# kirilllzaitsev/vision_mtl

Hardware: AMD Instinct MI355X
Metric: images/sec fwd+bwd, basic model 128x256 (higher is better)
Workload: dtype f32

## Files before the change

### include/vmtl.h

```cpp
#ifndef VMTL_H
#define VMTL_H

#ifdef __cplusplus
extern "C" {
#endif

#define VMTL_ACT_NONE 0
#define VMTL_ACT_RELU 1
#define VMTL_ACT_HSWISH 2
#define VMTL_ACT_HSIGMOID 3
#define VMTL_ACT_SIGMOID 4

#define VMTL_PREC_FP32 0
#define VMTL_PREC_BF16 1

const char* vmtl_version(void);
const char* vmtl_last_error_string(void);
int vmtl_reload_env(void);
int vmtl_timestamp(long long* out, void* stream);


int vmtl_conv2d_fwd(const float* x, const float* wp, const float* bias, float* y, float* stats,
                    int B, int H, int W, int Cs, int Ho, int Wo, int ldy, int Nw, int Cout,
                    int KH, int KW, int stride, int pad, int act, int shuffle, void* stream);
// ... 63 lines not shown
int vmtl_unpack_up2(const float* slabs, float* grad, int Cout, int Cos, int C0, int Cin, int nslabs, void* stream);

int vmtl_conv2d_wgrad_splits(int M, int Nw, int Ktot);
int vmtl_conv2d_wgrad(const float* x, const float* dy, float* slabs, int splits, int B, int H, int W, int Cs,
                      int Ho, int Wo, int ldy, int Nw, int KH, int KW, int stride, int pad, void* stream);
int vmtl_conv2d_wgrad_p(const float* x, const float* dy, float* slabs, int splits, int B, int H, int W, int Cs,
                        int Ho, int Wo, int ldy, int Nw, int KH, int KW, int stride, int pad, int precision,
                        void* stream);

int vmtl_conv3x3_wgrad_small_supported(int Cs, int ldy, int W);
int vmtl_conv3x3_wgrad_small_slabs(int B, int H, int W);
int vmtl_conv3x3_wgrad_small(const float* x, const float* dy, float* slabs, int nslabs, int B, int H, int W, int Cs,
                             int ldy, int Nw, void* stream);


int vmtl_conv3x3_small_supported(int Cs, int Nw);
int vmtl_conv3x3_small_tiles(int B, int H, int W);
int vmtl_conv3x3_small_stat_rows(int B, int H, int W);
int vmtl_conv3x3_small_stat_block(int B, int H, int W);
int vmtl_conv3x3_small(const float* x, const float* x2, const float* pa, const float* pb, const float* pc,
                       int act_in, float* a_out, const float* wp, const float* bias, float* y, float* yb, int Ca,
                       float* stats, int ep_mode, const float* ez_x, const float* ez_mean, const float* ez_invstd,
                       const float* ez_gamma, const float* ez_beta, int ez_act, int B, int H, int W, int Cs, int ldy,
                       int Nw, int Cout, void* stream);

int vmtl_conv3x3_halo_supported(int B, int H, int W, int Cs, int ldy, int Nw);
int vmtl_conv3x3_halo_stat_rows(int B, int H, int W);
int vmtl_conv3x3_halo_stat_block(int B, int H, int W);
int vmtl_conv3x3_halo(const float* x, const float* pa, const float* pc, int act_in, float* a_out, const float* wp,
                      const float* bias, float* y, float* stats, int ep_mode, const float* ez_x, const float* ez_mean,
                      const float* ez_invstd, const float* ez_gamma, const float* ez_beta, int ez_act, int B, int H,
                      int W, int Cs, int ldy, int Nw, int Cout, void* stream);

int vmtl_dwconv_fwd(const float* x, const float* wp, float* y, int B, int H, int W, int Cs, int Ho, int Wo,
                    int K, int stride, int pad, void* stream);
int vmtl_dwconv_bn_stats_rows(int M, int Cs);
int vmtl_dwconv_bn_stats_block(int M, int Cs);
int vmtl_dwconv_bn_fwd(const float* x, const float* coef_a, const float* coef_c, int act, const float* wp, float* y,
                       float* a_out, float* partial, int B, int H, int W, int Cs, int Ho, int Wo, int K, int stride,
                       int pad, void* stream);
int vmtl_dwconv_bwd_data(const float* dy, const float* wp, float* dx, int B, int H, int W, int Cs, int Ho,
                         int Wo, int K, int stride, int pad, void* stream);
int vmtl_dwconv_bwd_data_add(const float* dy, const float* wp, const float* addend, float* dx, int B, int H, int W,
                             int Cs, int Ho, int Wo, int K, int stride, int pad, void* stream);
int vmtl_dwconv_bwd_weight_rows(int M, int Cs);
int vmtl_dwconv_bwd_weight(const float* x, const float* dy, float* partial, float* dw, int B, int H, int W,
                           int C, int Cs, int Ho, int Wo, int K, int stride, int pad, void* stream);

int vmtl_pack_weights(const float* src, float* dst, int R1, int R0, int T, int C, int Cs, long long sr1,
                      long long sr0, long long st, long long sc, int flip, void* stream);
int vmtl_pack_weights_scaled(const float* src, float* dst, int R1, int R0, int T, int C, int Cs, long long sr1,
                             long long sr0, long long st, long long sc, int flip, const float* scale, int sstride,
                             int smode, void* stream);
int vmtl_unpack_weights_stitch(const float* packed, float* grad, const float* w, const float* scale, int sstride,
                               float* ds, float* work, int R0, int T, int C, int Cs, int nslabs, long long slab_stride,
                               int reduce_all, void* stream);
int vmtl_pack_desc_bytes(void);
int vmtl_pack_weights_batch(const void* descs, int n, long long total, void* stream);
int vmtl_pack_weights_slice(const float* src, float* dst, int R0, int T, int C, int group, long long sr0,
                            long long st, long long sc, int flip, void* stream);
int vmtl_unpack_weights(const float* packed, float* grad, int R1, int R0, int T, int C, int Cs,
                        long long sr1, long long sr0, long long st, long long sc, int flip, int nslabs,
                        long long slab_stride, void* stream);

int vmtl_reduce_rows(int M);
int vmtl_bn_stats(const float* x, int M, int C, int Cs, float* partial, int nblk_from_conv,
                  int rows_per_blk_from_conv, float eps, float momentum, float* running_mean, float* running_var, long long* num_batches_tracked,
                  float* save_mean, float* save_invstd, void* stream);
int vmtl_bn_eval_stats(const float* running_mean, const float* running_var, int C, int Cs, float eps,
                       float* save_mean, float* save_invstd, void* stream);
int vmtl_bn_stats_coef(const float* x, int M, int C, int Cs, float* partial, int nblk_from_conv,
                       int rows_per_blk_from_conv, float eps, float momentum, float* running_mean, float* running_var,
                       long long* num_batches_tracked, float* save_mean, float* save_invstd, const float* gamma,
                       const float* beta, float* coef_a, float* coef_c, void* stream);
int vmtl_bn_eval_stats_coef(const float* running_mean, const float* running_var, int C, int Cs, float eps,
                            float* save_mean, float* save_invstd, const float* gamma, const float* beta,
                            float* coef_a, float* coef_c, void* stream);
int vmtl_bn_eval_desc_bytes(void);
int vmtl_bn_eval_stats_batch(const void* descs, int n, int max_cs, void* stream);
int vmtl_bn_apply(const float* x, const float* mean, const float* invstd, const float* gamma,
                  const float* beta, const float* mul, const float* res, float* y, long long M, int C,
                  int Cs, int act, void* stream);
int vmtl_bn_fuse_max_rows(void);
int vmtl_bn_apply_fused(const float* x, const float* partial, int nblk, int rows_per_blk, float eps, float momentum,
                        float* running_mean, float* running_var, long long* num_batches_tracked, float* save_mean,
                        float* save_invstd, const float* gamma, const float* beta, const float* mul, const float* res,
                        float* y, long long M, int C, int Cs, int act, void* stream);
int vmtl_bn_bwd(const float* x, const float* dy, const float* mean, const float* invstd, const float* gamma,
                const float* beta, const float* mul, float* dmul, float* partial, float* sum_dz,
                float* sum_dzx, float* dx, int M, int C, int Cs, int act, int training, void* stream);
int vmtl_bn_bwd_finalize(const float* partial, int nblk, int M, int C, int Cs, float* sum_dz, float* sum_dzx,
                         const float* mean, const float* invstd, const float* gamma, int training, float* coef_a,
                         float* coef_b, float* coef_c, void* stream);
int vmtl_bn_bwd_apply(const float* x, const float* dz, const float* mean, const float* invstd, const float* gamma,
                      const float* sum_dz, const float* sum_dzx, float* dx, int M, int C, int Cs, int training,
                      void* stream);

int vmtl_bn_act_pool2_fwd(const float* x, const float* mean, const float* invstd, const float* gamma,
                          const float* beta, float* y, int B, int H, int W, int C, int Cs, int act, void* stream);
int vmtl_bn_act_pool2_bwd(const float* x, const float* dyp, const float* mean, const float* invstd,
                          const float* gamma, const float* beta, float* partial, float* sum_dz, float* sum_dzx,
                          float* dx, int B, int H, int W, int C, int Cs, int act, int training, void* stream);

int vmtl_conv2d_dgrad_s2_supported(int K, int pad);
long long vmtl_conv2d_dgrad_s2_ws(int B, int H, int W, int Cs, int Ho, int Wo, int ldy, int K, int pad);
long long vmtl_pack_dgrad_s2_size(int Cin, int ldy, int K, int pad);
int vmtl_pack_dgrad_s2(const float* w, float* dst, int Cout, int Cin, int ldy, int K, int pad, void* stream);
int vmtl_conv2d_dgrad_s2(const float* dy, const float* wp, float* dx, float* ws, int B, int H, int W, int Cs, int Ho,
                         int Wo, int ldy, int Cin, int K, int pad, void* stream);
int vmtl_conv2d_dgrad_s2_p(const float* dy, const float* wp, float* dx, float* ws, int B, int H, int W, int Cs, int Ho,
                           int Wo, int ldy, int Cin, int K, int pad, int precision, void* stream);
int vmtl_bn_act_pool3s2_fwd(const float* x, const float* mean, const float* invstd, const float* gamma,
                            const float* beta, float* a_out, float* y, unsigned char* idx, int B, int H, int W, int C,
                            int Cs, int act, void* stream);
int vmtl_bn_act_pool3s2_bwd(const float* x, const float* dskip, const float* dyp, const unsigned char* idx,
                            const float* mean, const float* invstd, const float* gamma, const float* beta, float* dz,
                            float* partial, float* sum_dz, float* sum_dzx, float* dx, int B, int H, int W, int C, int Cs,
                            int act, int training, void* stream);
int vmtl_bn_add_act_fwd(const float* z, const float* mean_a, const float* invstd_a, const float* gamma_a,
                        const float* beta_a, const float* res, const float* zd, const float* mean_b, const float* invstd_b,
                        const float* gamma_b, const float* beta_b, float* y, int M, int C, int Cs, int act, void* stream);
int vmtl_bn_add_act_bwd(const float* z, const float* mean_a, const float* invstd_a, const float* gamma_a,
                        const float* beta_a, const float* res, const float* zd, const float* mean_b, const float* invstd_b,
                        const float* gamma_b, const float* beta_b, const float* dy, float* g, float* partial,
                        float* sum_dz_a, float* sum_dzx_a, float* sum_dz_b, float* sum_dzx_b, float* dz, float* dzd, int M,
                        int C, int Cs, int act, int training, void* stream);

int vmtl_colsum(const float* a, const float* b, int M, int C, int Cs, int mode, int reduce_all,
                float* partial, float* out, void* stream);

int vmtl_concat2(const float* a, int Ha, int Wa, int Ca, int Csa, int upa, int oha, int owa,
                 const float* b, int Hb, int Wb, int Cb, int Csb, int upb, int ohb, int owb, float* y,
                 int B, int H, int W, int Cd, void* stream);
int vmtl_concat2_bwd(const float* dy, float* dx, int B, int H, int W, int Cd, int c_off, int Hs, int Ws,
                     int C, int Cs, int up, int oh, int ow, void* stream);
int vmtl_maxpool2_fwd(const float* x, float* y, int B, int H, int W, int Cs, void* stream);
int vmtl_maxpool2_bwd(const float* x, const float* dy, float* dx, int B, int H, int W, int Cs, void* stream);
int vmtl_bilinear_up2_fwd(const float* x, float* y, int B, int H, int W, int Cs, void* stream);
int vmtl_bilinear_up2_bwd(const float* dy, float* dx, int B, int H, int W, int Cs, void* stream);
int vmtl_spatial_mean(const float* x, float* y, int B, int HW, int Cs, void* stream);
int vmtl_channel_bcast(const float* x, const float* s, float* y, int B, int HW, int Cs, int mode, void* stream);
int vmtl_channel_scale_bwd_s(const float* x, const float* dy, float* ds, int B, int HW, int Cs, void* stream);
int vmtl_fc_max_rows(void);
int vmtl_fc_fwd(const float* a, int a_parts, long long a_part_stride, float a_scale, const float* a_z, int a_act,
                float* a_out, const float* w, const float* bias, float* z, float* y, int M, int K, int N, int lda,
                int ldw, int ldy, int act, void* stream);
int vmtl_fc_wgrad(const float* x, int x_parts, long long x_part_stride, float x_scale, const float* dyo, int dy_parts,
                  long long dy_part_stride, const float* zo, float* dw, float* db, int M, int K, int N, int lda, int ldn,
                  int act, void* stream);
int vmtl_hw_reduce_parts(int B, int HW, int Cs);
int vmtl_hw_reduce(const float* x, const float* y, float* part, int B, int HW, int Cs, void* stream);
int vmtl_channel_scale_add(const float* x, const float* s, const float* t, float t_scale, float* y, int B, int HW,
                           int Cs, void* stream);
int vmtl_stitch(const float* x, const float* w, float* y, long long M, int C, int Cs, int wstride, void* stream);
int vmtl_stitch_bwd(const float* x, const float* dy, const float* w, float* dx, float* partial, float* dw, int M,
                    int C, int Cs, int wstride, int reduce_all, void* stream);
int vmtl_eltwise(const float* a, const float* b, float* y, int mode, long long total, void* stream);
int vmtl_add_n(const float* a, const float* b, const float* c, const float* d, float* y, long long total, void* stream);
int vmtl_axpby(const float* a, const float* b, float* y, float wa, float wb, long long total, void* stream);
int vmtl_fill_zero(float* p, long long n, void* stream);
int vmtl_argmax_channels(const float* z, long long* out, int B, int HW, int C, long long sb, long long sc,
                         long long sp, void* stream);
int vmtl_nchw_to_nhwc(const float* x, float* y, int B, int C, int HW, int Cs, int Cw, void* stream);
int vmtl_nhwc_to_nchw(const float* x, float* y, int B, int C, int HW, int Cs, void* stream);
int vmtl_hwc_to_nhwc_pad(const float* x, float* y, long long P, int C, int Cs, float scale, void* stream);
#define VMTL_DEPTH_U16 0
#define VMTL_DEPTH_I32 1
int vmtl_nyuv2_resize_parts(int B, int Hi, int Wi, int Ho, int Wo, int depth_dtype);
int vmtl_nyuv2_resize(const void* img, const void* mask, const void* depth, int depth_dtype, float* img_out,
                      long long* mask_out, float* depth_out, float* part, int B, int Hi, int Wi, int Ho, int Wo,
                      float max_depth, void* stream);

long long vmtl_ce_workspace_bytes(long long P);
int vmtl_ce_fwd(const float* logits, const long long* target, float* loss, void* workspace, int B, int HW,
                int C, long long sb, long long sc, long long sp, void* stream);
int vmtl_ce_fwd_argmax(const float* logits, const long long* target, float* loss, void* workspace,
                       long long* argmax, int B, int HW, int C, long long sb, long long sc, long long sp,
                       void* stream);
int vmtl_ce_bwd(const float* logits, const long long* target, const float* grad_out, float* dlogits, int B,
                int HW, int C, long long sb, long long sc, long long sp, void* stream);
int vmtl_ce_bwd_strided(const float* logits, const long long* target, const float* grad_out, float* dlogits, int B,
                        int HW, int C, long long sb, long long sc, long long sp, long long dsb, long long dsc,
                        long long dsp, void* stream);
long long vmtl_silog_workspace_bytes(long long P);
int vmtl_silog_fwd(const float* pred, const float* target, float min_depth, float* loss, float* stats,
                   void* workspace, long long P, void* stream);
int vmtl_silog_bwd(const float* pred, const float* target, const float* stats, const float* grad_out,
                   float min_depth, float* dpred, long long P, void* stream);
int vmtl_l1_fwd(const float* pred, const float* target, float* loss, void* workspace, long long P, void* stream);
int vmtl_l1_bwd(const float* pred, const float* target, const float* grad_out, float* dpred, long long P,
                void* stream);

int vmtl_confusion_matrix(const long long* pred, const long long* target, int* cm, long long P, int C,
                          void* stream);
int vmtl_segm_metrics(const int* cm, int C, float beta, float* out, void* stream);

int vmtl_adam_step(float* p, const float* g, float* m, float* v, const float* step_ptr, float lr, float b1,
                   float b2, float eps, float weight_decay, float grad_scale, long long n, void* stream);

#ifdef __cplusplus
}
#endif
#endif
```

### vision_mtl_amd/csrc/fc.hip

```cpp
#include "common.h"

struct FcP {
  const float* a;
  const float* a_z;
  const float* w;
  const float* bias;
  float* a_out;
  float* z;
  float* y;
  long long a_part_stride;
  float a_scale;
  int a_parts, a_act;
  int M, K, N, lda, ldw, ldy, act;
};

#define FC_WAVES 8
#define FC_UNROLL 4

template <int MT>
__global__ __launch_bounds__(FC_WAVES * 64) void fc_kernel(FcP p) {
  __shared__ f32x4 red[FC_WAVES][MT][64];
  const int tid = threadIdx.x, lane = tid & 63, wv = tid >> 6;
  const int l15 = lane & 15, lq = lane >> 4;
  const int n0 = blockIdx.x * 16;
  const int n = n0 + l15;
  f32x4 acc[MT];
#pragma unroll
  for (int t = 0; t < MT; ++t) acc[t] = (f32x4){0.f, 0.f, 0.f, 0.f};
  const int nchunks = (p.K + 15) >> 4;
  const bool wvec = (p.ldw & 3) == 0;
  for (int c0 = wv; c0 < nchunks; c0 += FC_WAVES * FC_UNROLL) {
    f32x4 fb[FC_UNROLL], fa[FC_UNROLL][MT];
#pragma unroll
    for (int u = 0; u < FC_UNROLL; ++u) {
      const int c = c0 + u * FC_WAVES;
      const int k4 = c * 16 + lq * 4;
      fb[u] = (f32x4){0.f, 0.f, 0.f, 0.f};
      if (c < nchunks && n < p.N && k4 < p.K) {
        const float* wp = p.w + (size_t)n * p.ldw + k4;
        if (wvec && k4 + 3 < p.K) {
          fb[u] = *reinterpret_cast<const f32x4*>(wp);
        } else {
#pragma unroll
          for (int e = 0; e < 4; ++e)
            if (k4 + e < p.K) fb[u][e] = wp[e];
        }
      }
#pragma unroll
      for (int t = 0; t < MT; ++t) {
        const int m = t * 16 + l15;
        f32x4 v = {0.f, 0.f, 0.f, 0.f};
        if (c < nchunks && m < p.M && k4 < p.lda) {
          const float* ap = p.a + (size_t)m * p.lda + k4;
          v = *reinterpret_cast<const f32x4*>(ap);
          for (int s = 1; s < p.a_parts; ++s) v += *reinterpret_cast<const f32x4*>(ap + s * p.a_part_stride);
          v *= p.a_scale;
          if (p.a_out != nullptr && (c % (int)gridDim.x) == (int)blockIdx.x)
            *reinterpret_cast<f32x4*>(p.a_out + (size_t)m * p.lda + k4) = v;
          if (p.a_z != nullptr) {
            const f32x4 zv = *reinterpret_cast<const f32x4*>(p.a_z + (size_t)m * p.lda + k4);
#pragma unroll
            for (int e = 0; e < 4; ++e) v[e] *= act_grad(zv[e], p.a_act);
          }
        }
        fa[u][t] = v;
      }
    }
#pragma unroll
    for (int u = 0; u < FC_UNROLL; ++u)
#pragma unroll
      for (int t = 0; t < MT; ++t)
#pragma unroll
        for (int e = 0; e < 4; ++e)
          acc[t] = __builtin_amdgcn_mfma_f32_16x16x4f32(fa[u][t][e], fb[u][e], acc[t], 0, 0, 0);
  }
#pragma unroll
  for (int t = 0; t < MT; ++t) red[wv][t][lane] = acc[t];
  __syncthreads();
  if (tid >= 512) return;
  const int ln = tid & 63, rg = (tid >> 6) & 3, rt = tid >> 8;
  const int col = ln & 15, row = 4 * (ln >> 4) + rg;
  const int nn = n0 + col;
  if (nn >= p.ldy) return;
  const float bv = (p.bias != nullptr && nn < p.N) ? p.bias[nn] : 0.f;
  for (int t = rt; t < MT; t += 2) {
    const int m = t * 16 + row;
    if (m >= p.M) continue;
    const float* r0 = reinterpret_cast<const float*>(&red[0][t][ln]) + rg;
    constexpr int WS = MT * 64 * 4;
    float v = bv;
#pragma unroll
    for (int w = 0; w < FC_WAVES; ++w) v += r0[w * WS];
    if (nn >= p.N) v = 0.f;
    if (p.z != nullptr) p.z[(size_t)m * p.ldy + nn] = v;
    p.y[(size_t)m * p.ldy + nn] = nn < p.N ? act_fwd(v, p.act) : 0.f;
  }
}

extern "C" int vmtl_fc_max_rows() { return 64; }

extern "C" int vmtl_fc_fwd(const float* a, int a_parts, long long a_part_stride, float a_scale, const float* a_z,
                           int a_act, float* a_out, const float* w, const float* bias, float* z, float* y, int M,
                           int K, int N, int lda, int ldw, int ldy, int act, void* stream) {
  VMTL_ENTER();
  if (!a || !w || !y || M <= 0 || M > 64 || K <= 0 || N <= 0 || (lda & 3) || lda < K || ldw < K || ldy < N ||
      a_parts < 1 || (a_parts > 1 && (a_part_stride & 3)))
    return VMTL_ERR_ARG;
  FcP p{a, a_z, w, bias, a_out, z, y, a_part_stride, a_scale, a_parts, a_act, M, K, N, lda, ldw, ldy, act};
  const dim3 grid(cdiv(ldy, 16));
  hipStream_t st = (hipStream_t)stream;
  switch (cdiv(M, 16)) {
    case 1: hipLaunchKernelGGL(fc_kernel<1>, grid, dim3(FC_WAVES * 64), 0, st, p); break;
    case 2: hipLaunchKernelGGL(fc_kernel<2>, grid, dim3(FC_WAVES * 64), 0, st, p); break;
    case 3: hipLaunchKernelGGL(fc_kernel<3>, grid, dim3(FC_WAVES * 64), 0, st, p); break;
    default: hipLaunchKernelGGL(fc_kernel<4>, grid, dim3(FC_WAVES * 64), 0, st, p); break;
  }
  return vmtl_check_launch();
}

struct FcWgP {
  const float* x;
  const float* dyo;
  const float* zo;
  float* dw;
  float* db;
  long long x_part_stride, dy_part_stride;
  float x_scale;
  int x_parts, dy_parts, M, K, N, lda, ldn, act;
};

__global__ __launch_bounds__(256) void fc_wgrad_kernel(FcWgP p) {
  __shared__ float dz[64][8];
  const int tid = threadIdx.x;
  const int n0 = blockIdx.x * 8;
  for (int idx = tid; idx < p.M * 8; idx += 256) {
    const int m = idx >> 3, i = idx & 7, n = n0 + i;
    float v = 0.f;
    if (n < p.N) {
      const size_t off = (size_t)m * p.ldn + n;
      v = p.dyo[off];
      for (int s = 1; s < p.dy_parts; ++s) v += p.dyo[off + s * p.dy_part_stride];
      if (p.zo != nullptr) v *= act_grad(p.zo[off], p.act);
    }
    dz[m][i] = v;
  }
  __syncthreads();
  for (int k = tid; k < p.K; k += 256) {
    float acc[8];
#pragma unroll
    for (int i = 0; i < 8; ++i) acc[i] = 0.f;
    for (int mb = 0; mb < p.M; mb += 8) {
      float xv[8];
#pragma unroll
      for (int u = 0; u < 8; ++u) {
        xv[u] = 0.f;
        if (mb + u < p.M) {
          const size_t off = (size_t)(mb + u) * p.lda + k;
          xv[u] = p.x[off];
          for (int s = 1; s < p.x_parts; ++s) xv[u] += p.x[off + s * p.x_part_stride];
        }
      }
#pragma unroll
      for (int u = 0; u < 8; ++u) {
        if (mb + u < p.M) {
          const float x1 = xv[u] * p.x_scale;
#pragma unroll
          for (int i = 0; i < 8; ++i) acc[i] += dz[mb + u][i] * x1;
        }
      }
    }
#pragma unroll
    for (int i = 0; i < 8; ++i)
      if (n0 + i < p.N) p.dw[(size_t)(n0 + i) * p.K + k] = acc[i];
  }
  if (p.db != nullptr && tid < 8 && n0 + tid < p.N) {
    float s = 0.f;
    for (int m = 0; m < p.M; ++m) s += dz[m][tid];
    p.db[n0 + tid] = s;
  }
}

extern "C" int vmtl_fc_wgrad(const float* x, int x_parts, long long x_part_stride, float x_scale, const float* dyo,
                             int dy_parts, long long dy_part_stride, const float* zo, float* dw, float* db, int M,
                             int K, int N, int lda, int ldn, int act, void* stream) {
  VMTL_ENTER();
  if (!x || !dyo || !dw || M <= 0 || M > 64 || K <= 0 || N <= 0 || lda < K || ldn < N || x_parts < 1 || dy_parts < 1)
    return VMTL_ERR_ARG;
  FcWgP p{x, dyo, zo, dw, db, x_part_stride, dy_part_stride, x_scale, x_parts, dy_parts, M, K, N, lda, ldn, act};
  hipLaunchKernelGGL(fc_wgrad_kernel, dim3(cdiv(N, 8)), dim3(256), 0, (hipStream_t)stream, p);
  return vmtl_check_launch();
}

__global__ __launch_bounds__(256) void hw_reduce_kernel(const float* __restrict__ x, const float* __restrict__ y,
                                                        float* __restrict__ part, int B, int HW, int Cs, int rows_per) {
  __shared__ f32x4 red[256];
  const int CQ = Cs >> 2;
  const int cq = min(CQ, 256);
  const int RP = 256 / cq;
  const int tid = threadIdx.x;
  const int ql = tid % cq, rg = tid / cq;
  const int q = blockIdx.x * 256 + ql;
  const int b = blockIdx.y, s = blockIdx.z;
  const int r_begin = s * rows_per, r_end = min(HW, r_begin + rows_per);
  f32x4 acc = {0.f, 0.f, 0.f, 0.f};
  if (rg < RP && q < CQ) {
    const float* xb = x + (size_t)b * HW * Cs + (size_t)q * 4;
    const float* yb = y != nullptr ? y + (size_t)b * HW * Cs + (size_t)q * 4 : nullptr;
    f32x4 a1 = {0.f, 0.f, 0.f, 0.f}, a2 = a1, a3 = a1;
    int r = r_begin + rg;
    for (; r + 3 * RP < r_end; r += 4 * RP) {
      f32x4 v0 = *reinterpret_cast<const f32x4*>(xb + (size_t)r * Cs);
      f32x4 v1 = *reinterpret_cast<const f32x4*>(xb + (size_t)(r + RP) * Cs);
      f32x4 v2 = *reinterpret_cast<const f32x4*>(xb + (size_t)(r + 2 * RP) * Cs);
      f32x4 v3 = *reinterpret_cast<const f32x4*>(xb + (size_t)(r + 3 * RP) * Cs);
      if (yb != nullptr) {
        v0 *= *reinterpret_cast<const f32x4*>(yb + (size_t)r * Cs);
        v1 *= *reinterpret_cast<const f32x4*>(yb + (size_t)(r + RP) * Cs);
        v2 *= *reinterpret_cast<const f32x4*>(yb + (size_t)(r + 2 * RP) * Cs);
        v3 *= *reinterpret_cast<const f32x4*>(yb + (size_t)(r + 3 * RP) * Cs);
      }
      acc += v0;
      a1 += v1;
      a2 += v2;
      a3 += v3;
    }
    for (; r < r_end; r += RP) {
      f32x4 v = *reinterpret_cast<const f32x4*>(xb + (size_t)r * Cs);
      if (yb != nullptr) v *= *reinterpret_cast<const f32x4*>(yb + (size_t)r * Cs);
      acc += v;
    }
    acc += a1 + (a2 + a3);
  }
  red[tid] = acc;
  __syncthreads();
  if (rg == 0 && q < CQ) {
    f32x4 t = red[ql];
    for (int g = 1; g < RP; ++g) t += red[g * cq + ql];
    *reinterpret_cast<f32x4*>(part + ((size_t)s * B + b) * Cs + (size_t)q * 4) = t;
  }
}

extern "C" int vmtl_hw_reduce_parts(int B, int HW, int Cs) {
  if (B <= 0 || HW <= 0 || Cs <= 0) return 0;
  const int cols = cdiv(Cs >> 2, 256);
  int want = cdiv(128, B * cols);
  int cap = cdiv(HW, 32);
  int S = want < cap ? want : cap;
  if (S < 1) S = 1;
  if (S > 32) S = 32;
  return cdiv(HW, cdiv(HW, S));
}

extern "C" int vmtl_hw_reduce(const float* x, const float* y, float* part, int B, int HW, int Cs, void* stream) {
  VMTL_ENTER();
  if (!x || !part || (Cs & 3) || B <= 0 || HW <= 0) return VMTL_ERR_ARG;
  const int S = vmtl_hw_reduce_parts(B, HW, Cs);
  const int rows_per = cdiv(HW, S);
  hipLaunchKernelGGL(hw_reduce_kernel, dim3(cdiv(Cs >> 2, 256), B, S), dim3(256), 0, (hipStream_t)stream, x, y, part, B,
                     HW, Cs, rows_per);
  return vmtl_check_launch();
}

__global__ __launch_bounds__(256) void channel_scale_add_kernel(const float* __restrict__ x, const float* __restrict__ s,
                                                                const float* __restrict__ t, float t_scale,
                                                                float* __restrict__ y, int HW, int Cs, long long total4) {
  const int CQ = Cs >> 2;
  for (long long i = (long long)blockIdx.x * 256 + threadIdx.x; i < total4; i += (long long)gridDim.x * 256) {
    const int q = (int)(i % CQ);
    const int b = (int)(i / ((long long)CQ * HW));
    f32x4 v = reinterpret_cast<const f32x4*>(x)[i] * *reinterpret_cast<const f32x4*>(s + (size_t)b * Cs + (size_t)q * 4);
    if (t != nullptr) v += *reinterpret_cast<const f32x4*>(t + (size_t)b * Cs + (size_t)q * 4) * t_scale;
    reinterpret_cast<f32x4*>(y)[i] = v;
  }
}

extern "C" int vmtl_channel_scale_add(const float* x, const float* s, const float* t, float t_scale, float* y, int B,
                                      int HW, int Cs, void* stream) {
  VMTL_ENTER();
  if (!x || !s || !y || (Cs & 3) || B <= 0 || HW <= 0) return VMTL_ERR_ARG;
  const long long total4 = (long long)B * HW * (Cs >> 2);
  long long blocks = (total4 + 255) / 256;
  if (blocks > 4096) blocks = 4096;
  hipLaunchKernelGGL(channel_scale_add_kernel, dim3((unsigned)blocks), dim3(256), 0, (hipStream_t)stream, x, s, t, t_scale,
                     y, HW, Cs, total4);
  return vmtl_check_launch();
}
```

### vision_mtl_amd/ops.py

```python
from __future__ import annotations

import contextlib
import os
import weakref
from typing import NamedTuple

import torch

from ._lib import lib
from .precision import conv_prec_code

ACT_NONE, ACT_RELU, ACT_HSWISH, ACT_HSIGMOID, ACT_SIGMOID = 0, 1, 2, 3, 4
ACT_CODES = {None: 0, "none": 0, "relu": 1, "hardswish": 2, "hardsigmoid": 3, "sigmoid": 4}


def ceil4(c: int) -> int:
    return (c + 3) // 4 * 4


def _stream() -> int:
    return torch.cuda.current_stream().cuda_stream


def _req(t: torch.Tensor, name: str = "tensor") -> torch.Tensor:
# ... 1626 lines not shown
class _Concat2(torch.autograd.Function):
    @staticmethod
    def forward(ctx, a, b, Ca, Cb, up_a, up_b, H, W, off_a, off_b):
        a = _req(a, "a")
        B, Ha, Wa, Csa = a.shape
        if b is not None:
            b = _req(b, "b")
            _, Hb, Wb, Csb = b.shape
        else:
            Hb = Wb = Csb = 0
            Cb = 0
        Cd = ceil4(Ca + Cb)
        y = _empty((B, H, W, Cd), a)
        _k("vmtl_concat2", a=a, Ha=Ha, Wa=Wa, Ca=Ca, Csa=Csa, upa=up_a, oha=off_a[0], owa=off_a[1], b=b, Hb=Hb, Wb=Wb,
           Cb=Cb, Csb=Csb, upb=up_b, ohb=off_b[0], owb=off_b[1], y=y, B=B, H=H, W=W, Cd=Cd)
        ctx.cfg = (a.shape, None if b is None else b.shape, Ca, Cb, up_a, up_b, H, W, off_a, off_b)
        return y

    @staticmethod
    def backward(ctx, dy):
        ashape, bshape, Ca, Cb, up_a, up_b, H, W, off_a, off_b = ctx.cfg
        dy = _req(dy, "dy")
        B, _, _, Cd = dy.shape
        da = db = None
        if ctx.needs_input_grad[0]:
            da = _empty(ashape, dy)
            _k("vmtl_concat2_bwd", dy=dy, dx=da, B=B, H=H, W=W, Cd=Cd, c_off=0, Hs=ashape[1], Ws=ashape[2], C=Ca,
               Cs=ashape[3], up=up_a, oh=off_a[0], ow=off_a[1])
        if bshape is not None and ctx.needs_input_grad[1]:
            db = _empty(bshape, dy)
            _k("vmtl_concat2_bwd", dy=dy, dx=db, B=B, H=H, W=W, Cd=Cd, c_off=Ca, Hs=bshape[1], Ws=bshape[2], C=Cb,
               Cs=bshape[3], up=up_b, oh=off_b[0], ow=off_b[1])
        return da, db, None, None, None, None, None, None, None, None


def concat2(a, Ca, b=None, Cb=0, up_a=1, up_b=1, out_hw=None, off_a=(0, 0), off_b=(0, 0)):
    if out_hw is None:
        out_hw = (a.shape[1] * up_a, a.shape[2] * up_a)
    return _Concat2.apply(a, b, Ca, Cb, up_a, up_b, out_hw[0], out_hw[1], tuple(off_a), tuple(off_b))


class _MaxPool2(torch.autograd.Function):
    @staticmethod
    def forward(ctx, x):
        x = _req(x, "x")
        B, H, W, Cs = x.shape
        y = _empty((B, H // 2, W // 2, Cs), x)
        _k("vmtl_maxpool2_fwd", x=x, y=y, B=B, H=H, W=W, Cs=Cs)
        ctx.save_for_backward(x)
        return y

    @staticmethod
    def backward(ctx, dy):
        (x,) = ctx.saved_tensors
        dy = _req(dy, "dy")
        B, H, W, Cs = x.shape
        dx = _empty(x.shape, x)
        _k("vmtl_maxpool2_bwd", x=x, dy=dy, dx=dx, B=B, H=H, W=W, Cs=Cs)
        return dx


def maxpool2(x):
    return _MaxPool2.apply(x)


class _BilinearUp2(torch.autograd.Function):
    @staticmethod
    def forward(ctx, x):
        x = _req(x, "x")
        B, H, W, Cs = x.shape
        y = _empty((B, 2 * H, 2 * W, Cs), x)
        _k("vmtl_bilinear_up2_fwd", x=x, y=y, B=B, H=H, W=W, Cs=Cs)
        ctx.shape = x.shape
        return y

    @staticmethod
    def backward(ctx, dy):
        dy = _req(dy, "dy")
        B, H, W, Cs = ctx.shape
        dx = _empty(ctx.shape, dy)
        _k("vmtl_bilinear_up2_bwd", dy=dy, dx=dx, B=B, H=H, W=W, Cs=Cs)
        return dx


def bilinear_up2(x):
    return _BilinearUp2.apply(x)


class _SpatialMean(torch.autograd.Function):
    @staticmethod
    def forward(ctx, x):
        x = _req(x, "x")
        B, H, W, Cs = x.shape
        y = _empty((B, 1, 1, Cs), x)
        _k("vmtl_spatial_mean", x=x, y=y, B=B, HW=H * W, Cs=Cs)
        ctx.shape = x.shape
        return y

    @staticmethod
    def backward(ctx, dy):
        dy = _req(dy, "dy")
        B, H, W, Cs = ctx.shape
        dx = _empty(ctx.shape, dy)
        _k("vmtl_channel_bcast", x=None, s=dy, y=dx, B=B, HW=H * W, Cs=Cs, mode=1)
        return dx


def spatial_mean(x):
    return _SpatialMean.apply(x)


class _ChannelScale(torch.autograd.Function):
    @staticmethod
    def forward(ctx, x, s):
        x, s = _req(x, "x"), _req(s, "s")
        B, H, W, Cs = x.shape
        y = _empty(x.shape, x)
        _k("vmtl_channel_bcast", x=x, s=s, y=y, B=B, HW=H * W, Cs=Cs, mode=0)
        ctx.save_for_backward(x, s)
        return y

    @staticmethod
    def backward(ctx, dy):
        x, s = ctx.saved_tensors
        dy = _req(dy, "dy")
        B, H, W, Cs = x.shape
        dx = ds = None
        if ctx.needs_input_grad[0]:
            dx = _empty(x.shape, x)
            _k("vmtl_channel_bcast", x=dy, s=s, y=dx, B=B, HW=H * W, Cs=Cs, mode=0)
        if ctx.needs_input_grad[1]:
            ds = _empty(s.shape, x)
            _k("vmtl_channel_scale_bwd_s", x=x, dy=dy, ds=ds, B=B, HW=H * W, Cs=Cs)
        return dx, ds


def channel_scale(x, s):
    return _ChannelScale.apply(x, s)


class _SqueezeExcite(torch.autograd.Function):

    @staticmethod
    def forward(ctx, x, wr, br, we, be, act1, act2):
        x, wr, we = _req(x, "x"), _req(wr, "reduce weight"), _req(we, "expand weight")
        B, H, W, Cs = x.shape
        HW = H * W
        R, C = wr.shape[0], wr.shape[1]
        if ceil4(C) != Cs or tuple(we.shape[:2]) != (C, R) or br is None or be is None:
            raise ValueError("squeeze_excite: weights must be (R, C, 1, 1) / (C, R, 1, 1) with biases, matching x")
        if B > lib().raw("vmtl_fc_max_rows")():
            raise ValueError("squeeze_excite: batch too large for the batch-sized GEMM kernels")
        Rs = ceil4(R)
        S = lib().raw("vmtl_hw_reduce_parts")(B, HW, Cs)
        parts = _empty((S, B, Cs), x)
        _k("vmtl_hw_reduce", x=x, y=None, part=parts, B=B, HW=HW, Cs=Cs)
        z1, h = _empty((B, Rs), x), _empty((B, Rs), x)
        pooled = _empty((B, Cs), x)
        _k("vmtl_fc_fwd", a=parts, a_parts=S, a_part_stride=B * Cs, a_scale=1.0 / HW, a_z=None, a_act=0, a_out=pooled,
           w=wr, bias=br, z=z1, y=h, M=B, K=C, N=R, lda=Cs, ldw=C, ldy=Rs, act=act1)
        z2, g = _empty((B, Cs), x), _empty((B, Cs), x)
        _k("vmtl_fc_fwd", a=h, a_parts=1, a_part_stride=0, a_scale=1.0, a_z=None, a_act=0, a_out=None, w=we, bias=be,
           z=z2, y=g, M=B, K=R, N=C, lda=Rs, ldw=R, ldy=Cs, act=act2)
        y = _empty(x.shape, x)
        _k("vmtl_channel_scale_add", x=x, s=g, t=None, t_scale=0.0, y=y, B=B, HW=HW, Cs=Cs)
        ctx.save_for_backward(x, pooled, z1, h, z2, g, wr, we)
        ctx.S = S
        ctx.acts = (act1, act2)
        ctx.slots = (_slot(wr), _slot(br), _slot(we), _slot(be))
        return y

    @staticmethod
    def backward(ctx, dy):
        x, pooled, z1, h, z2, g, wr, we = ctx.saved_tensors
        act1, act2 = ctx.acts
        dy = _req(dy, "dy")
        B, H, W, Cs = x.shape
        HW = H * W
        R, C = wr.shape[0], wr.shape[1]
        Rs, S = ceil4(R), ctx.S
        dparts = _empty((S, B, Cs), x)
        _k("vmtl_hw_reduce", x=dy, y=x, part=dparts, B=B, HW=HW, Cs=Cs)
        weT = packs.get(we, "dgrad", (1, R, 1, C, Cs, 0, 1, 1, R, 1))
        dh = _empty((B, Rs), x)
        dg = _empty((B, Cs), x)
        _k("vmtl_fc_fwd", a=dparts, a_parts=S, a_part_stride=B * Cs, a_scale=1.0, a_z=z2, a_act=act2, a_out=dg, w=weT,
           bias=None, z=None, y=dh, M=B, K=C, N=R, lda=Cs, ldw=Cs, ldy=Rs, act=0)
        fork = side.mark()
        dx = None
        if ctx.needs_input_grad[0]:
            wrT = packs.get(wr, "dgrad", (1, C, 1, R, Rs, 0, 1, 1, C, 1))
            dmean = _empty((B, Cs), x)
            _k("vmtl_fc_fwd", a=dh, a_parts=1, a_part_stride=0, a_scale=1.0, a_z=z1, a_act=act1, a_out=None, w=wrT,
               bias=None, z=None, y=dmean, M=B, K=R, N=C, lda=Rs, ldw=Rs, ldy=Cs, act=0)
            dx = _empty(x.shape, x)
            _k("vmtl_channel_scale_add", x=dy, s=g, t=dmean, t_scale=1.0 / HW, y=dx, B=B, HW=HW, Cs=Cs)
        slots = ctx.slots
        all_slots = all(s is not None for s in slots)
        with side.branch(all_slots, B, fork, dg, dh, pooled, z1, h, z2):
            dwr = _empty(wr.shape, x) if slots[0] is None else slots[0]
            dbr = _empty((R,), x) if slots[1] is None else slots[1]
            dwe = _empty(we.shape, x) if slots[2] is None else slots[2]
            dbe = _empty((C,), x) if slots[3] is None else slots[3]
            _k("vmtl_fc_wgrad", x=h, x_parts=1, x_part_stride=0, x_scale=1.0, dyo=dg, dy_parts=1, dy_part_stride=0,
               zo=z2, dw=dwe, db=dbe, M=B, K=R, N=C, lda=Rs, ldn=Cs, act=act2)
            _k("vmtl_fc_wgrad", x=pooled, x_parts=1, x_part_stride=0, x_scale=1.0, dyo=dh, dy_parts=1,
               dy_part_stride=0, zo=z1, dw=dwr, db=dbr, M=B, K=C, N=R, lda=Cs, ldn=Rs, act=act1)
        ret = [None if sl is not None else t for t, sl in zip((dwr, dbr, dwe, dbe), slots)]
        return dx, ret[0], ret[1], ret[2], ret[3], None, None


def squeeze_excite(x, w_reduce, b_reduce, w_expand, b_expand, act1=ACT_RELU, act2=ACT_HSIGMOID):
    return _SqueezeExcite.apply(x, w_reduce, b_reduce, w_expand, b_expand, act1, act2)


def squeeze_excite_max_batch() -> int:
    return lib().raw("vmtl_fc_max_rows")()


class _Stitch(torch.autograd.Function):

    @staticmethod
    def forward(ctx, x, weights, task, C):
        x = _req(x, "x")
        weights = _req(weights, "weights")
        B, H, W, Cs = x.shape
        T = weights.shape[0]
        channel_wise = weights.dim() == 3
        off = (task * T + task) * (weights.shape[2] if channel_wise else 1)
        wview = weights.view(-1)[off:]
        y = _empty(x.shape, x)
        _k("vmtl_stitch", _flop=8.0 * B * H * W * C, x=x, w=wview, y=y, M=B * H * W, C=C, Cs=Cs, wstride=1 if channel_wise else 0)
        ctx.save_for_backward(x, weights)
        ctx.cfg = (task, C, channel_wise, off)
        ctx.slot = _slot(weights)
        return y

    @staticmethod
    def backward(ctx, dy):
        x, weights = ctx.saved_tensors
        task, C, channel_wise, off = ctx.cfg
        dy = _req(dy, "dy")
        B, H, W, Cs = x.shape
        M = B * H * W
        dx = dw = None
        wv = weights.view(-1)[off:]
        ws = 1 if channel_wise else 0
        if ctx.needs_input_grad[1]:
            n = C if channel_wise else 1
            if ctx.slot is not None:
                out = ctx.slot.view(-1)[off:off + n]
            else:
                dw = torch.zeros_like(weights)
                out = dw.view(-1)[off:off + n]
            dx = _empty(x.shape, x) if ctx.needs_input_grad[0] else None
            _k("vmtl_stitch_bwd", x=x, dy=dy, w=wv, dx=dx, partial=_empty((_reduce_rows(M) + 1, Cs), x), dw=out, M=M, C=C, Cs=Cs,
               wstride=ws, reduce_all=0 if channel_wise else 1)
        elif ctx.needs_input_grad[0]:
            dx = _empty(x.shape, x)
            _k("vmtl_stitch", x=dy, w=wv, y=dx, M=M, C=C, Cs=Cs, wstride=ws)
        return dx, dw, None, None


def stitch(x, weights, task, C):
    return _Stitch.apply(x, weights, task, C)


class _ToNHWC(torch.autograd.Function):

    @staticmethod
    def forward(ctx, x):
        x = _req(x, "x")
        B, C, H, W = x.shape
        Cs = ceil4(C)
        y = _empty((B, H, W, Cs), x)
        _k("vmtl_nchw_to_nhwc", x=x, y=y, B=B, C=C, HW=H * W, Cs=Cs, Cw=Cs)
        ctx.C = C
        return y

    @staticmethod
    def backward(ctx, dy):
        dy = _req(dy, "dy")
        B, H, W, Cs = dy.shape
        dx = _empty((B, ctx.C, H, W), dy)
        _k("vmtl_nhwc_to_nchw", x=dy, y=dx, B=B, C=ctx.C, HW=H * W, Cs=Cs)
        return dx


def to_nhwc(x):
    st = getattr(x, "_vmtl_nhwc", None)
    if st is not None and st.shape[0] == x.shape[0] and tuple(st.shape[1:3]) == tuple(x.shape[2:]) and not x.requires_grad:
        return st
    return _ToNHWC.apply(x)


def hwc_to_model_input(x_hwc, scale: float = 1.0):
    x_hwc = _req(x_hwc, "img")
    B, H, W, C = x_hwc.shape
    Cs = ceil4(C)
    st = _empty((B, H, W, Cs), x_hwc)
    _k("vmtl_hwc_to_nhwc_pad", x=x_hwc, y=st, P=B * H * W, C=C, Cs=Cs, scale=scale)
    view = st[..., :C].permute(0, 3, 1, 2)
    view._vmtl_nhwc = st
    return view



def _req_dtype(t: torch.Tensor, name: str, dtypes: tuple) -> torch.Tensor:
    if not t.is_cuda:
        raise RuntimeError(
            f"{name} is on {t.device}: the vmtl hot path only runs as HIP kernels on an MI355X "
            "(there is deliberately no CPU fallback)"
        )
    if t.dtype not in dtypes:
        raise TypeError(f"{name} must be one of {[str(d) for d in dtypes]}, got {t.dtype}")
    t = t if t.is_contiguous() else t.contiguous()
    return t if t.data_ptr() % 16 == 0 else t.clone()


DEPTH_DTYPES = {torch.uint16: 0, torch.int32: 1}


def nyuv2_resize(img, mask, depth, size, max_depth: float = 10.0):
    img = _req_dtype(img, "img", (torch.uint8,))
    mask = _req_dtype(mask, "mask", (torch.uint8,))
    depth = _req_dtype(depth, "depth", tuple(DEPTH_DTYPES))
    if img.dim() != 4 or img.shape[-1] != 3:
        raise ValueError(f"nyuv2_resize: img must be (B, H, W, 3), got {tuple(img.shape)}")
    B, Hi, Wi, _ = img.shape
    if tuple(mask.shape) != (B, Hi, Wi) or tuple(depth.shape) != (B, Hi, Wi):
        raise ValueError(f"nyuv2_resize: mask {tuple(mask.shape)} and depth {tuple(depth.shape)} must be {(B, Hi, Wi)}")
    Ho, Wo = (int(v) for v in size)
    code = DEPTH_DTYPES[depth.dtype]
    nparts = lib().raw("vmtl_nyuv2_resize_parts")(B, Hi, Wi, Ho, Wo, code)
    if nparts < 0:
        lib()._raise("vmtl_nyuv2_resize_parts", nparts)
    st = _empty((B, Ho, Wo, 4), img)
    m = torch.empty((B, Ho, Wo), dtype=torch.int64, device=img.device)
    d = _empty((B, Ho, Wo, 1), img)
    part = _empty((nparts,), img)
    _k("vmtl_nyuv2_resize", img=img, mask=mask, depth=depth, depth_dtype=code, img_out=st, mask_out=m, depth_out=d,
       part=part, B=B, Hi=Hi, Wi=Wi, Ho=Ho, Wo=Wo, max_depth=float(max_depth))
    view = st[..., :3].permute(0, 3, 1, 2)
    view._vmtl_nhwc = st
    return view, m, d

class _ToNCHW(torch.autograd.Function):

    @staticmethod
    def forward(ctx, x, C):
        x = _req(x, "x")
# ... 477 lines not shown
```

Baseline: 2631.

## Fuse squeeze-excite gate pooling and FC layers into per-image kernels

Adds fused per-image kernels for the squeeze-excite gate. The forward pass pools, runs both FC layers and applies the activations in one launch, and the backward pass computes the dy·x reduction plus both transposed matvecs in one launch. The two weight-gradient kernels are also merged into a single launch. This cuts kernel launches, partial-sum buffers and packed transposed weights. The cost is only B blocks for the spatial reduction, which may underuse the GPU on large feature maps; the forward fusion is limited to small weight matrices unless an env override is set.

```diff
diff --git a/include/vmtl.h b/include/vmtl.h
--- a/include/vmtl.h
+++ b/include/vmtl.h
@@ -239,6 +239,14 @@
 int vmtl_hw_reduce(const float* x, const float* y, float* part, int B, int HW, int Cs, void* stream);
 int vmtl_channel_scale_add(const float* x, const float* s, const float* t, float t_scale, float* y, int B, int HW,
                            int Cs, void* stream);
+int vmtl_se_gate_supported(int B, int C, int R);
+int vmtl_se_gate_fwd(const float* x, const float* wr, const float* br, const float* we, const float* be, float* pooled,
+                     float* z1, float* h, float* z2, float* g, int B, int HW, int C, int R, int act1, int act2,
+                     void* stream);
+int vmtl_se_gate_bwd(const float* dy, const float* x, const float* z1, const float* z2, const float* wr, const float* we,
+                     float* dg, float* dh, float* dmean, int B, int HW, int C, int R, int act1, int act2, void* stream);
+int vmtl_se_wgrad(const float* pooled, const float* h, const float* dg, const float* dh, const float* z1, const float* z2,
+                  float* dwr, float* dbr, float* dwe, float* dbe, int B, int C, int R, int act1, int act2, void* stream);
 int vmtl_stitch(const float* x, const float* w, float* y, long long M, int C, int Cs, int wstride, void* stream);
 int vmtl_stitch_bwd(const float* x, const float* dy, const float* w, float* dx, float* partial, float* dw, int M,
                     int C, int Cs, int wstride, int reduce_all, void* stream);
diff --git a/vision_mtl_amd/csrc/fc.hip b/vision_mtl_amd/csrc/fc.hip
--- a/vision_mtl_amd/csrc/fc.hip
+++ b/vision_mtl_amd/csrc/fc.hip
@@ -129,10 +129,10 @@
   int x_parts, dy_parts, M, K, N, lda, ldn, act;
 };
 
-__global__ __launch_bounds__(256) void fc_wgrad_kernel(FcWgP p) {
+__device__ __forceinline__ void fc_wgrad_block(const FcWgP& p, int bx) {
   __shared__ float dz[64][8];
   const int tid = threadIdx.x;
-  const int n0 = blockIdx.x * 8;
+  const int n0 = bx * 8;
   for (int idx = tid; idx < p.M * 8; idx += 256) {
     const int m = idx >> 3, i = idx & 7, n = n0 + i;
     float v = 0.f;
@@ -179,6 +179,8 @@
     p.db[n0 + tid] = s;
   }
 }
+
+__global__ __launch_bounds__(256) void fc_wgrad_kernel(FcWgP p) { fc_wgrad_block(p, blockIdx.x); }
 
 extern "C" int vmtl_fc_wgrad(const float* x, int x_parts, long long x_part_stride, float x_scale, const float* dyo,
                              int dy_parts, long long dy_part_stride, const float* zo, float* dw, float* db, int M,
@@ -285,3 +287,280 @@
                      y, HW, Cs, total4);
   return vmtl_check_launch();
 }
+
+#define SE_THREADS 1024
+#define SE_MAX_VEC 8192
+
+template <int V>
+__device__ __forceinline__ void se_ld(const float* p, float* o) {
+  if constexpr (V == 4) {
+    const f32x4 v = *reinterpret_cast<const f32x4*>(p);
+    o[0] = v[0], o[1] = v[1], o[2] = v[2], o[3] = v[3];
+  } else {
+    o[0] = p[0];
+  }
+}
+template <int V>
+__device__ __forceinline__ void se_st(float* p, const float* o) {
+  if constexpr (V == 4) {
+    *reinterpret_cast<f32x4*>(p) = (f32x4){o[0], o[1], o[2], o[3]};
+  } else {
+    p[0] = o[0];
+  }
+}
+
+template <int V, int MODE>
+__device__ __forceinline__ void se_colsum(const float* __restrict__ a, const float* __restrict__ b, const float* wv, int rows,
+                                          int cols, int ld, float* red, float* red2, float* out) {
+  const int tid = threadIdx.x;
+  const int ncg = cols / V;
+  for (int q0 = 0; q0 < ncg; q0 += SE_THREADS) {
+    const int cg = min(ncg - q0, SE_THREADS);
+    const int RP = SE_THREADS / cg;
+    const int ql = tid % cg, rg = tid / cg;
+    float acc[4][V];
+#pragma unroll
+    for (int u = 0; u < 4; ++u)
+#pragma unroll
+      for (int e = 0; e < V; ++e) acc[u][e] = 0.f;
+    if (rg < RP) {
+      const size_t col = (size_t)(q0 + ql) * V;
+      int r = rg;
+      for (; r + 3 * RP < rows; r += 4 * RP) {
+        float v[4][V];
+#pragma unroll
+        for (int u = 0; u < 4; ++u) se_ld<V>(a + (size_t)(r + u * RP) * ld + col, v[u]);
+        if constexpr (MODE == 1) {
+          float w[4][V];
+#pragma unroll
+          for (int u = 0; u < 4; ++u) se_ld<V>(b + (size_t)(r + u * RP) * ld + col, w[u]);
+#pragma unroll
+          for (int u = 0; u < 4; ++u)
+#pragma unroll
+            for (int e = 0; e < V; ++e) v[u][e] *= w[u][e];
+        }
+#pragma unroll
+        for (int u = 0; u < 4; ++u) {
+          const float f = MODE == 2 ? wv[r + u * RP] : 1.f;
+#pragma unroll
+          for (int e = 0; e < V; ++e) acc[u][e] += MODE == 2 ? v[u][e] * f : v[u][e];
+        }
+      }
+      for (; r < rows; r += RP) {
+        float v[V];
+        se_ld<V>(a + (size_t)r * ld + col, v);
+        if constexpr (MODE == 1) {
+          float w[V];
+          se_ld<V>(b + (size_t)r * ld + col, w);
+#pragma unroll
+          for (int e = 0; e < V; ++e) v[e] *= w[e];
+        }
+        const float f = MODE == 2 ? wv[r] : 1.f;
+#pragma unroll
+        for (int e = 0; e < V; ++e) acc[0][e] += MODE == 2 ? v[e] * f : v[e];
+      }
+#pragma unroll
+      for (int e = 0; e < V; ++e) acc[0][e] += acc[1][e] + (acc[2][e] + acc[3][e]);
+    }
+    se_st<V>(red + (size_t)tid * V, acc[0]);
+    __syncthreads();
+    const int G = min(RP, 8);
+    if (rg < G) {
+      float t[V];
+      se_ld<V>(red + (size_t)(rg * cg + ql) * V, t);
+      for (int g = rg + G; g < RP; g += G) {
+        float v[V];
+        se_ld<V>(red + (size_t)(g * cg + ql) * V, v);
+#pragma unroll
+        for (int e = 0; e < V; ++e) t[e] += v[e];
+      }
+      se_st<V>(red2 + (size_t)(rg * cg + ql) * V, t);
+    }
+    __syncthreads();
+    if (rg == 0) {
+      float t[V];
+      se_ld<V>(red2 + (size_t)ql * V, t);
+      for (int g = 1; g < G; ++g) {
+        float v[V];
+        se_ld<V>(red2 + (size_t)(g * cg + ql) * V, v);
+#pragma unroll
+        for (int e = 0; e < V; ++e) t[e] += v[e];
+      }
+      se_st<V>(out + (size_t)(q0 + ql) * V, t);
+    }
+    __syncthreads();
+  }
+}
+
+template <int V, class F>
+__device__ __forceinline__ void se_rowdot(const float* __restrict__ w, int rows, int K, const float* v, F fin) {
+  const int tid = threadIdx.x;
+  const int KG = K / V;
+  int LPR = 1;
+  while (LPR < KG && LPR < 16) LPR <<= 1;
+  const int l = tid & (LPR - 1), rl = tid / LPR, RIF = SE_THREADS / LPR;
+  for (int n0 = 0; n0 < rows; n0 += RIF) {
+    const int n = n0 + rl;
+    float acc[4] = {0.f, 0.f, 0.f, 0.f};
+    if (n < rows) {
+      const float* wp = w + (size_t)n * K;
+      for (int k = l; k < KG; k += 4 * LPR) {
+        float wv[4][V];
+#pragma unroll
+        for (int u = 0; u < 4; ++u) se_ld<V>(wp + (size_t)min(k + u * LPR, KG - 1) * V, wv[u]);
+#pragma unroll
+        for (int u = 0; u < 4; ++u) {
+          const int kk = k + u * LPR;
+          if (kk < KG) {
+#pragma unroll
+            for (int e = 0; e < V; ++e) acc[u] += wv[u][e] * v[kk * V + e];
+          }
+        }
+      }
+    }
+    float s = (acc[0] + acc[1]) + (acc[2] + acc[3]);
+    for (int o = LPR >> 1; o > 0; o >>= 1) s += __shfl_xor(s, o, 64);
+    if (l == 0 && n < rows) fin(n, s);
+  }
+}
+
+struct SeFwdP {
+  const float *x, *wr, *br, *we, *be;
+  float *pooled, *z1, *h, *z2, *g;
+  int HW, C, R, Cs, Rs, act1, act2, vec_r, vec_e;
+};
+
+__global__ __launch_bounds__(SE_THREADS) void se_gate_fwd_kernel(SeFwdP p) {
+  extern __shared__ float se_vec[];
+  __shared__ f32x4 red4[SE_THREADS], red24[SE_THREADS];
+  float* red = reinterpret_cast<float*>(red4);
+  float* red2 = reinterpret_cast<float*>(red24);
+  float* vc = se_vec;
+  float* vr = se_vec + p.Cs;
+  const int tid = threadIdx.x, b = blockIdx.x;
+  se_colsum<4, 0>(p.x + (size_t)b * p.HW * p.Cs, nullptr, nullptr, p.HW, p.Cs, p.Cs, red, red2, vc);
+  const float inv = 1.f / (float)p.HW;
+  for (int c = tid; c < p.Cs; c += SE_THREADS) {
+    const float m = vc[c] * inv;
+    vc[c] = m;
+    p.pooled[(size_t)b * p.Cs + c] = m;
+  }
+  for (int r = p.R + tid; r < p.Rs; r += SE_THREADS) {
+    vr[r] = 0.f;
+    p.z1[(size_t)b * p.Rs + r] = 0.f;
+    p.h[(size_t)b * p.Rs + r] = 0.f;
+  }
+  for (int c = p.C + tid; c < p.Cs; c += SE_THREADS) {
+    p.z2[(size_t)b * p.Cs + c] = 0.f;
+    p.g[(size_t)b * p.Cs + c] = 0.f;
+  }
+  __syncthreads();
+  auto fin1 = [&](int n, float s) {
+    const float z = s + p.br[n];
+    const float hv = act_fwd(z, p.act1);
+    p.z1[(size_t)b * p.Rs + n] = z;
+    p.h[(size_t)b * p.Rs + n] = hv;
+    vr[n] = hv;
+  };
+  if (p.vec_r) se_rowdot<4>(p.wr, p.R, p.C, vc, fin1);
+  else se_rowdot<1>(p.wr, p.R, p.C, vc, fin1);
+  __syncthreads();
+  auto fin2 = [&](int n, float s) {
+    const float z = s + p.be[n];
+    p.z2[(size_t)b * p.Cs + n] = z;
+    p.g[(size_t)b * p.Cs + n] = act_fwd(z, p.act2);
+  };
+  if (p.vec_e) se_rowdot<4>(p.we, p.C, p.R, vr, fin2);
+  else se_rowdot<1>(p.we, p.C, p.R, vr, fin2);
+}
+
+struct SeBwdP {
+  const float *dy, *x, *z1, *z2, *wr, *we;
+  float *dg, *dh, *dmean;
+  int HW, C, R, Cs, Rs, act1, act2, vec_r, vec_e;
+};
+
+__global__ __launch_bounds__(SE_THREADS) void se_gate_bwd_kernel(SeBwdP p) {
+  extern __shared__ float se_vec[];
+  __shared__ f32x4 red4[SE_THREADS], red24[SE_THREADS];
+  float* red = reinterpret_cast<float*>(red4);
+  float* red2 = reinterpret_cast<float*>(red24);
+  float* vc = se_vec;
+  float* vr = se_vec + p.Cs;
+  const int tid = threadIdx.x, b = blockIdx.x;
+  const size_t img = (size_t)b * p.HW * p.Cs;
+  se_colsum<4, 1>(p.dy + img, p.x + img, nullptr, p.HW, p.Cs, p.Cs, red, red2, vc);
+  for (int c = tid; c < p.Cs; c += SE_THREADS) {
+    const float d = vc[c];
+    p.dg[(size_t)b * p.Cs + c] = d;
+    vc[c] = c < p.C ? d * act_grad(p.z2[(size_t)b * p.Cs + c], p.act2) : 0.f;
+  }
+  __syncthreads();
+  if (p.vec_e) se_colsum<4, 2>(p.we, nullptr, vc, p.C, p.R, p.R, red, red2, vr);
+  else se_colsum<1, 2>(p.we, nullptr, vc, p.C, p.R, p.R, red, red2, vr);
+  for (int r = tid; r < p.Rs; r += SE_THREADS) {
+    const float d = r < p.R ? vr[r] : 0.f;
+    p.dh[(size_t)b * p.Rs + r] = d;
+    vr[r] = r < p.R ? d * act_grad(p.z1[(size_t)b * p.Rs + r], p.act1) : 0.f;
+  }
+  if (p.dmean == nullptr) return;
+  __syncthreads();
+  if (p.vec_r) se_colsum<4, 2>(p.wr, nullptr, vr, p.R, p.C, p.C, red, red2, vc);
+  else se_colsum<1, 2>(p.wr, nullptr, vr, p.R, p.C, p.C, red, red2, vc);
+  for (int c = tid; c < p.Cs; c += SE_THREADS) p.dmean[(size_t)b * p.Cs + c] = c < p.C ? vc[c] : 0.f;
+}
+
+__global__ __launch_bounds__(256) void se_wgrad_kernel(FcWgP pe, FcWgP pr, int nbe) {
+  if ((int)blockIdx.x < nbe) fc_wgrad_block(pe, blockIdx.x);
+  else fc_wgrad_block(pr, blockIdx.x - nbe);
+}
+
+static inline int ceil4i(int c) { return (c + 3) & ~3; }
+static inline bool se_vec_ok(const float* w, int ld) { return (ld & 3) == 0 && ((uintptr_t)w & 15) == 0; }
+static inline bool se_shape_ok(int B, int HW, int C, int R) {
+  return B > 0 && B <= 64 && HW > 0 && C > 0 && R > 0 && ceil4i(C) + ceil4i(R) <= SE_MAX_VEC;
+}
+
+#define SE_FWD_MAX_WEIGHTS 16384
+extern "C" int vmtl_se_gate_supported(int B, int C, int R) {
+  static EnvInt e{"VMTL_SE_FUSED", 1};
+  const int mode = env_int(e);
+  if (mode == 0 || !se_shape_ok(B, 1, C, R)) return 0;
+  return 1 | ((mode >= 2 || (long long)C * R <= SE_FWD_MAX_WEIGHTS) ? 2 : 0);
+}
+
+extern "C" int vmtl_se_gate_fwd(const float* x, const float* wr, const float* br, const float* we, const float* be,
+                                float* pooled, float* z1, float* h, float* z2, float* g, int B, int HW, int C, int R,
+                                int act1, int act2, void* stream) {
+  VMTL_ENTER();
+  if (!x || !wr || !br || !we || !be || !pooled || !z1 || !h || !z2 || !g || !se_shape_ok(B, HW, C, R)) return VMTL_ERR_ARG;
+  const int Cs = ceil4i(C), Rs = ceil4i(R);
+  SeFwdP p{x, wr, br, we, be, pooled, z1, h, z2, g, HW, C, R, Cs, Rs, act1, act2, se_vec_ok(wr, C), se_vec_ok(we, R)};
+  hipLaunchKernelGGL(se_gate_fwd_kernel, dim3(B), dim3(SE_THREADS), (Cs + Rs) * sizeof(float), (hipStream_t)stream, p);
+  return vmtl_check_launch();
+}
+
+extern "C" int vmtl_se_gate_bwd(const float* dy, const float* x, const float* z1, const float* z2, const float* wr,
+                                const float* we, float* dg, float* dh, float* dmean, int B, int HW, int C, int R, int act1,
+                                int act2, void* stream) {
+  VMTL_ENTER();
+  if (!dy || !x || !z1 || !z2 || !wr || !we || !dg || !dh || !se_shape_ok(B, HW, C, R)) return VMTL_ERR_ARG;
+  const int Cs = ceil4i(C), Rs = ceil4i(R);
+  SeBwdP p{dy, x, z1, z2, wr, we, dg, dh, dmean, HW, C, R, Cs, Rs, act1, act2, se_vec_ok(wr, C), se_vec_ok(we, R)};
+  hipLaunchKernelGGL(se_gate_bwd_kernel, dim3(B), dim3(SE_THREADS), (Cs + Rs) * sizeof(float), (hipStream_t)stream, p);
+  return vmtl_check_launch();
+}
+
+extern "C" int vmtl_se_wgrad(const float* pooled, const float* h, const float* dg, const float* dh, const float* z1,
+                             const float* z2, float* dwr, float* dbr, float* dwe, float* dbe, int B, int C, int R,
+                             int act1, int act2, void* stream) {
+  VMTL_ENTER();
+  if (!pooled || !h || !dg || !dh || !z1 || !z2 || !dwr || !dwe || B <= 0 || B > 64 || C <= 0 || R <= 0)
+    return VMTL_ERR_ARG;
+  const int Cs = ceil4i(C), Rs = ceil4i(R);
+  FcWgP pe{h, dg, z2, dwe, dbe, 0, 0, 1.f, 1, 1, B, R, C, Rs, Cs, act2};
+  FcWgP pr{pooled, dh, z1, dwr, dbr, 0, 0, 1.f, 1, 1, B, C, R, Cs, Rs, act1};
+  const int nbe = cdiv(C, 8);
+  hipLaunchKernelGGL(se_wgrad_kernel, dim3(nbe + cdiv(R, 8)), dim3(256), 0, (hipStream_t)stream, pe, pr, nbe);
+  return vmtl_check_launch();
+}
diff --git a/vision_mtl_amd/ops.py b/vision_mtl_amd/ops.py
--- a/vision_mtl_amd/ops.py
+++ b/vision_mtl_amd/ops.py
@@ -1802,6 +1802,19 @@
         if B > lib().raw("vmtl_fc_max_rows")():
             raise ValueError("squeeze_excite: batch too large for the batch-sized GEMM kernels")
         Rs = ceil4(R)
+        ctx.acts = (act1, act2)
+        ctx.slots = (_slot(wr), _slot(br), _slot(we), _slot(be))
+        route = lib().raw("vmtl_se_gate_supported")(B, C, R)
+        ctx.fused = bool(route & 1)
+        if route & 2:
+            pooled, z1, h = _empty((B, Cs), x), _empty((B, Rs), x), _empty((B, Rs), x)
+            z2, g = _empty((B, Cs), x), _empty((B, Cs), x)
+            _k("vmtl_se_gate_fwd", x=x, wr=wr, br=br, we=we, be=be, pooled=pooled, z1=z1, h=h, z2=z2, g=g, B=B, HW=HW,
+               C=C, R=R, act1=act1, act2=act2)
+            y = _empty(x.shape, x)
+            _k("vmtl_channel_scale_add", x=x, s=g, t=None, t_scale=0.0, y=y, B=B, HW=HW, Cs=Cs)
+            ctx.save_for_backward(x, pooled, z1, h, z2, g, wr, we)
+            return y
         S = lib().raw("vmtl_hw_reduce_parts")(B, HW, Cs)
         parts = _empty((S, B, Cs), x)
         _k("vmtl_hw_reduce", x=x, y=None, part=parts, B=B, HW=HW, Cs=Cs)
@@ -1816,8 +1829,6 @@
         _k("vmtl_channel_scale_add", x=x, s=g, t=None, t_scale=0.0, y=y, B=B, HW=HW, Cs=Cs)
         ctx.save_for_backward(x, pooled, z1, h, z2, g, wr, we)
         ctx.S = S
-        ctx.acts = (act1, act2)
-        ctx.slots = (_slot(wr), _slot(br), _slot(we), _slot(be))
         return y
 
     @staticmethod
@@ -1828,7 +1839,29 @@
         B, H, W, Cs = x.shape
         HW = H * W
         R, C = wr.shape[0], wr.shape[1]
-        Rs, S = ceil4(R), ctx.S
+        Rs = ceil4(R)
+        slots = ctx.slots
+        all_slots = all(s is not None for s in slots)
+        if ctx.fused:
+            dg, dh = _empty((B, Cs), x), _empty((B, Rs), x)
+            dmean = _empty((B, Cs), x) if ctx.needs_input_grad[0] else None
+            _k("vmtl_se_gate_bwd", dy=dy, x=x, z1=z1, z2=z2, wr=wr, we=we, dg=dg, dh=dh, dmean=dmean, B=B, HW=HW, C=C, R=R,
+               act1=act1, act2=act2)
+            fork = side.mark()
+            dx = None
+            if dmean is not None:
+                dx = _empty(x.shape, x)
+                _k("vmtl_channel_scale_add", x=dy, s=g, t=dmean, t_scale=1.0 / HW, y=dx, B=B, HW=HW, Cs=Cs)
+            with side.branch(all_slots, B, fork, dg, dh, pooled, z1, h, z2):
+                dwr = _empty(wr.shape, x) if slots[0] is None else slots[0]
+                dbr = _empty((R,), x) if slots[1] is None else slots[1]
+                dwe = _empty(we.shape, x) if slots[2] is None else slots[2]
+                dbe = _empty((C,), x) if slots[3] is None else slots[3]
+                _k("vmtl_se_wgrad", pooled=pooled, h=h, dg=dg, dh=dh, z1=z1, z2=z2, dwr=dwr, dbr=dbr, dwe=dwe, dbe=dbe,
+                   B=B, C=C, R=R, act1=act1, act2=act2)
+            ret = [None if sl is not None else t for t, sl in zip((dwr, dbr, dwe, dbe), slots)]
+            return dx, ret[0], ret[1], ret[2], ret[3], None, None
+        S = ctx.S
         dparts = _empty((S, B, Cs), x)
         _k("vmtl_hw_reduce", x=dy, y=x, part=dparts, B=B, HW=HW, Cs=Cs)
         weT = packs.get(we, "dgrad", (1, R, 1, C, Cs, 0, 1, 1, R, 1))
@@ -1845,8 +1878,6 @@
                bias=None, z=None, y=dmean, M=B, K=R, N=C, lda=Rs, ldw=Rs, ldy=Cs, act=0)
             dx = _empty(x.shape, x)
             _k("vmtl_channel_scale_add", x=dy, s=g, t=dmean, t_scale=1.0 / HW, y=dx, B=B, HW=HW, Cs=Cs)
-        slots = ctx.slots
-        all_slots = all(s is not None for s in slots)
         with side.branch(all_slots, B, fork, dg, dh, pooled, z1, h, z2):
             dwr = _empty(wr.shape, x) if slots[0] is None else slots[0]
             dbr = _empty((R,), x) if slots[1] is None else slots[1]
```

Result: faster. 2663 (median of 6 runs) (+1.2%).
